# mbilos/stribor

Measured on AMD Instinct MI355X. Metric: log_prob samples/sec, D=64 8-layer affine-coupling, higher is better.
Workload: dtype f32

## Files before the change

stribor_amd/csrc/sx_flow_kernel.h:

```cpp
#pragma once
#include "sx_common.h"
#include "sx_flow_types.h"
#include "sx_cubic_core.h"
#include "sx_pointwise_core.h"
#include <stdlib.h>
#include <type_traits>

#define SX_HALF_LOG_2PI 0.91893853320467274178f

#ifdef SX_F16X3
#define SX_PREC_NS sx_f16x3
#else
#define SX_PREC_NS sx_f32x
#endif
namespace SX_PREC_NS {

__host__ __device__ static inline int sx_kmap(int r, int h) { return (r & 3) + 8 * (r >> 2) + 4 * h; }

extern __shared__ __attribute__((aligned(16))) float smem[];

typedef __attribute__((address_space(3))) void lds_void;

template <int NS>
struct tile {
// ... 419 lines not shown
#define SX_PIN_ACC(a) asm volatile("" : "+v"(a))
template <int NS, bool PIN = true, class F>
__device__ __forceinline__ void gemm_tile_pf(const char *wb, afr &cur, int next_off, const btile<NS> &b, tile<NS> &acc, F &&f) {
    afr nxt = cur;
    if (next_off >= 0) nxt = afr_load(wb, next_off);
    __builtin_amdgcn_sched_barrier(0);
#pragma unroll
    for (int s = 0; s < 2; ++s) {
        const h8 ah = __builtin_bit_cast(h8, cur.q[2 * s]), al = __builtin_bit_cast(h8, cur.q[2 * s + 1]);
#pragma unroll
        for (int n = 0; n < NS; ++n) { acc.v[n] = __builtin_amdgcn_mfma_f32_32x32x16_f16(al, b.hi[n][s], acc.v[n], 0, 0, 0); if constexpr (PIN) SX_PIN_ACC(acc.v[n]); }
        f(8 * s + 0); f(8 * s + 1); f(8 * s + 2);
        __builtin_amdgcn_sched_barrier(0);
#pragma unroll
        for (int n = 0; n < NS; ++n) { acc.v[n] = __builtin_amdgcn_mfma_f32_32x32x16_f16(ah, b.lo[n][s], acc.v[n], 0, 0, 0); if constexpr (PIN) SX_PIN_ACC(acc.v[n]); }
        f(8 * s + 3); f(8 * s + 4); f(8 * s + 5);
        __builtin_amdgcn_sched_barrier(0);
#pragma unroll
        for (int n = 0; n < NS; ++n) { acc.v[n] = __builtin_amdgcn_mfma_f32_32x32x16_f16(ah, b.hi[n][s], acc.v[n], 0, 0, 0); if constexpr (PIN) SX_PIN_ACC(acc.v[n]); }
        f(8 * s + 6); f(8 * s + 7);
        __builtin_amdgcn_sched_barrier(0);
    }
    cur = nxt;
}
__device__ __forceinline__ float pinned(float v) { asm volatile("" : "+v"(v)); return v; }
template <int NS, bool TRACK>
__device__ __forceinline__ void split_pair(const tile<NS> &c, u32x4 (&hi)[NS][2], u32x4 (&lo)[NS][2], int p, float &mx) {
#pragma unroll
    for (int n = 0; n < NS; ++n) {
        const float v0 = c.v[n][2 * p], v1 = c.v[n][2 * p + 1];
        if constexpr (TRACK) mx = rng_max(mx, v0, v1);
        const uint32_t ph = pk_f16(v0, v1);
        hi[n][p >> 2][p & 3] = ph;
        lo[n][p >> 2][p & 3] = pk_residual(ph, v0, v1);
    }
}
template <int NS>
__device__ __forceinline__ btile<NS> btile_of(const u32x4 (&hi)[NS][2], const u32x4 (&lo)[NS][2]) {
    btile<NS> b;
#pragma unroll
    for (int n = 0; n < NS; ++n)
#pragma unroll
        for (int s = 0; s < 2; ++s) { b.hi[n][s] = __builtin_bit_cast(h8, hi[n][s]); b.lo[n][s] = __builtin_bit_cast(h8, lo[n][s]); }
    return b;
}
template <int NS, int TX, int HT, int C0, int CT, int T0, int TT, bool REV>
__device__ __forceinline__ void coupling_affine_pf(tile<NS> (&xs)[TX], const wptr w, const dstep &st, float (&ldj)[NS],
                                                   rng_t &rg) {
    static_assert(CT == 2 && HT <= 2, "coupling_affine_pf: two conditioner tiles, hidden <= 64");
    constexpr int a2 = HT * CT * 1024 + HT * 32;
    constexpr int b2 = a2 + 2 * TT * HT * 1024;
    constexpr int bias1 = HT * CT * 1024;
    constexpr int NH = HT * CT, NO = 2 * TT * HT;
    auto off_of = [](int q) { return q < NH ? q * 1024 : (q < NH + NO ? a2 + (((q - NH) % (2 * TT)) * HT + (q - NH) / (2 * TT)) * 1024 : -1); };
    auto none = [](int) {};
    afr cur = afr_load(w.wb, 0);
    float mx = 0.f;
    u32x4 shi[NS][2], slo[NS][2];
    btile<NS> bsrc0 = make_btile_mx<NS>(xs[C0], mx);
    tile<NS> hid[HT];
    int q = 0;
    {
        tile<NS> acc = load_cfrag<NS>(w.cb, bias1);
        gemm_tile_pf<NS>(w.wb, cur, off_of(q + 1), bsrc0, acc, [&](int i) { if (!(i & 1)) split_pair<NS, true>(xs[C0 + 1], shi, slo, i >> 1, mx); });
        ++q;
        const btile<NS> bsrc1 = btile_of<NS>(shi, slo);
        gemm_tile_pf<NS>(w.wb, cur, off_of(q + 1), bsrc1, acc, none);
        ++q;
        hid[0] = acc;
        if constexpr (HT == 2) {
            tile<NS> acc1 = load_cfrag<NS>(w.cb, bias1 + 32);
            gemm_tile_pf<NS>(w.wb, cur, off_of(q + 1), bsrc0, acc1, [&](int i) {
                if (i & 1) return;
#pragma unroll
                for (int n = 0; n < NS; ++n) { hid[0].v[n][i] = pinned(fast_sig2(hid[0].v[n][i])); hid[0].v[n][i + 1] = pinned(fast_sig2(hid[0].v[n][i + 1])); }
            });
            ++q;
            gemm_tile_pf<NS>(w.wb, cur, off_of(q + 1), bsrc1, acc1, [&](int i) { if (!(i & 1)) split_pair<NS, false>(hid[0], shi, slo, i >> 1, mx); });
            ++q;
            hid[1] = acc1;
        }
        rng_note(rg, mx);
    }
    btile<NS> bh[HT];
    if constexpr (HT == 1) {
#pragma unroll
        for (int n = 0; n < NS; ++n)
#pragma unroll
            for (int r = 0; r < 16; r += 2) fast_sig2_pair(hid[0].v[n], r);
        bh[0] = make_btile<NS>(hid[0]);
    } else {
        bh[0] = btile_of<NS>(shi, slo);
    }
    f32x2 s[NS];
#pragma unroll
    for (int n = 0; n < NS; ++n) s[n] = f32x2{0.f, 0.f};
    tile<NS> out[2 * TT];
#pragma unroll
    for (int r = 0; r < 2 * TT; ++r) out[r] = load_cfrag<NS>(w.cb, b2 + r * 32);
    auto exp_rider = [&](tile<NS> &ls, int i) {
        if (i & 1) return;
#pragma unroll
        for (int n = 0; n < NS; ++n) {
            const float l0 = ls.v[n][i], l1 = ls.v[n][i + 1];
            s[n].x = pinned(s[n].x + l0);
            s[n].y = pinned(s[n].y + l1);
            ls.v[n][i] = pinned(__builtin_amdgcn_exp2f(l0));
            ls.v[n][i + 1] = pinned(__builtin_amdgcn_exp2f(l1));
        }
    };
    auto affine_rider = [&](tile<NS> &x, const tile<NS> &e, const tile<NS> &sh, int i) {
        if (i & 1) return;
#pragma unroll
        for (int n = 0; n < NS; ++n) {
            const f32x2 xv = {x.v[n][i], x.v[n][i + 1]}, sv = {sh.v[n][i], sh.v[n][i + 1]}, ev = {e.v[n][i], e.v[n][i + 1]};
            const f32x2 yv = REV ? pk_mul(pk_sub(xv, sv), ev) : pk_add(pk_mul(xv, ev), sv);
            x.v[n][i] = pinned(yv.x);
            x.v[n][i + 1] = pinned(yv.y);
        }
    };
#pragma unroll
    for (int k = 0; k < HT; ++k) {
#pragma unroll
        for (int r = 0; r < 2 * TT; ++r) {
            const bool last_k = k == HT - 1;
            gemm_tile_pf<NS>(w.wb, cur, off_of(q + 1), bh[k], out[r], [&](int i) {
                if (HT == 2 && k == 0) {
                    if (r == 0) {
                        if (!(i & 1)) {
#pragma unroll
                            for (int n = 0; n < NS; ++n) {
                                hid[HT - 1].v[n][i] = pinned(fast_sig2(hid[HT - 1].v[n][i]));
                                hid[HT - 1].v[n][i + 1] = pinned(fast_sig2(hid[HT - 1].v[n][i + 1]));
                            }
                        }
                    } else if (r <= 2) {
                        if ((i & 3) == 0) split_pair<NS, false>(hid[HT - 1], shi, slo, 4 * (r - 1) + (i >> 2), mx);
                    }
                }
                if (last_k) {
                    if (r & 1) exp_rider(out[r - 1], i);
                    else if (r >= 2) affine_rider(xs[T0 + r / 2 - 1], out[r - 2], out[r - 1], i);
                }
            });
            ++q;
            if (HT == 2 && k == 0 && r == 2) bh[1] = btile_of<NS>(shi, slo);
        }
    }
#pragma unroll
    for (int i = 0; i < 16; i += 2) affine_rider(xs[T0 + TT - 1], out[2 * TT - 2], out[2 * TT - 1], i);
#pragma unroll
    for (int n = 0; n < NS; ++n) ldj[n] += st.ldj_scale * (s[n].x + s[n].y);
}
#endif
template <int NS, int TX, int HT, int T0, int TT, bool REV>
__device__ __forceinline__ void coupling_affine_deep(tile<NS> (&xs)[TX], const tile<NS> (&hsrc)[HT], const wptr w,
                                                     const dstep &st, float (&ldj)[NS], rng_t &rg) {
    tile<NS> hid[HT];
    hidden_layer<NS, HT, HT, 0, HT, false>(hsrc, hid, w, 0, st.act, rg);
    constexpr int a2 = HT * HT * 1024 + HT * 32;
    constexpr int b2 = a2 + 2 * TT * HT * 1024;
    btile<NS> bh[HT];
#pragma unroll
    for (int m = 0; m < HT; ++m) bh[m] = make_btile<NS>(hid[m], rg);
    __builtin_amdgcn_sched_barrier(0);
    float s[NS];
#pragma unroll
    for (int n = 0; n < NS; ++n) s[n] = 0.f;
    const float sgn = REV ? -1.44269504088896341f : 1.44269504088896341f;
#pragma unroll
    for (int t = 0; t < TT; ++t) {
        tile<NS> ls = load_cfrag<NS>(w.cb, b2 + (2 * t) * 32);
        tile<NS> sh = load_cfrag<NS>(w.cb, b2 + (2 * t + 1) * 32);
#pragma unroll
        for (int m = 0; m < HT; ++m) {
            gemm_tile<NS>(w.wb, a2 + ((2 * t) * HT + m) * 1024, bh[m], ls);
            gemm_tile<NS>(w.wb, a2 + ((2 * t + 1) * HT + m) * 1024, bh[m], sh);
        }
        tile<NS> &x = xs[T0 + t];
#pragma unroll
        for (int n = 0; n < NS; ++n)
#pragma unroll
            for (int r = 0; r < 16; ++r) {
                s[n] += ls.v[n][r];
                const float e = __builtin_amdgcn_exp2f(ls.v[n][r] * sgn);
                x.v[n][r] = REV ? (x.v[n][r] - sh.v[n][r]) * e : x.v[n][r] * e + sh.v[n][r];
            }
    }
#pragma unroll
    for (int n = 0; n < NS; ++n) ldj[n] += st.ldj_scale * s[n];
}

template <int NS, int TX, int HT, int C0, int CT, int T0, int TT, bool REV, int PN>
__device__ __forceinline__ void coupling_affine_chunk(tile<NS> (&xs)[TX], tile<NS> (&pacc)[PN], const wptr w, const dstep &st,
                                                      float (&ldj)[NS], rng_t &rg) {
    tile<NS> hid[HT];
    hidden_layer<NS, TX, HT, C0, CT, true>(xs, hid, w, 0, SX_ACT_TANH_FOLDED, rg);
#pragma unroll
    for (int n = 0; n < NS; ++n)
#pragma unroll
        for (int r = 0; r < 16; r += 2) fast_sig2_pair(hid[HT - 1].v[n], r);
    btile<NS> bh[HT];
#pragma unroll
    for (int m = 0; m < HT; ++m) bh[m] = make_btile<NS>(hid[m]);
    __builtin_amdgcn_sched_barrier(0);
    constexpr int a2 = HT * CT * 1024 + HT * 32;
    constexpr int b2 = a2 + 2 * TT * HT * 1024;
    const bool first = st.pad & 1, last = st.pad & 2;
#pragma unroll
    for (int t = 0; t < 2 * TT; ++t) {
        tile<NS> acc = load_cfrag<NS>(w.cb, b2 + t * 32);
        if (!first) {
#pragma unroll
            for (int n = 0; n < NS; ++n)
#pragma unroll
                for (int r = 0; r < 16; ++r) acc.v[n][r] += pacc[t].v[n][r];
        }
#pragma unroll
        for (int m = 0; m < HT; ++m) gemm_tile<NS>(w.wb, a2 + (t * HT + m) * 1024, bh[m], acc);
        pacc[t] = acc;
    }
    if (last) {
#pragma unroll
        for (int t = 0; t < TT; ++t) {
            tile<NS> &x = xs[T0 + t];
#pragma unroll
            for (int n = 0; n < NS; ++n) {
                float s = 0.f;
#pragma unroll
                for (int r = 0; r < 16; ++r) {
                    const float l = pacc[2 * t].v[n][r], sh = pacc[2 * t + 1].v[n][r];
                    s += l;
                    const float e = __builtin_amdgcn_exp2f(l);
                    x.v[n][r] = REV ? (x.v[n][r] - sh) * e : x.v[n][r] * e + sh;
                }
                ldj[n] += st.ldj_scale * s;
            }
        }
    }
}
template <int NS, int TX, int HT, int C0, int CT, int T0, int TT, int PN>
__device__ __forceinline__ void coupling_affine_chunk_dispatch(tile<NS> (&xs)[TX], tile<NS> (&pacc)[PN], const wptr w, const dstep &st,
                                                               float (&ldj)[NS], rng_t &rg) {
    if (st.reverse) coupling_affine_chunk<NS, TX, HT, C0, CT, T0, TT, true>(xs, pacc, w, st, ldj, rg);
    else coupling_affine_chunk<NS, TX, HT, C0, CT, T0, TT, false>(xs, pacc, w, st, ldj, rg);
}

template <int TX, int HT, int C0>
__device__ __forceinline__ void wide_hidden(tile<1> (&xs)[TX], btile<1> (&bhp)[HT], const wptr w, rng_t &rg) {
    tile<1> hid[HT];
#ifdef SX_F16X3
    constexpr int CT = TX / 2;
    float mx = 0.f;
    btile<1> bsrc[CT];
#pragma unroll
    for (int c = 0; c < CT; ++c) bsrc[c] = make_btile_mx<1>(xs[C0 + c], mx);
    __builtin_amdgcn_sched_barrier(0);
    afr cura = afr_load(w.wb, 0);
    constexpr int bias = HT * CT * 1024;
#pragma unroll
    for (int m = 0; m < HT; ++m) {
        tile<1> acc = load_cfrag<1>(w.cb, bias + m * 32);
#pragma unroll
        for (int c = 0; c < CT; ++c) {
            const int qn = m * CT + c + 1;
            const int next_off = qn < HT * CT ? qn * 1024 : -1;
            if (m > 0 && c == 0)
                gemm_tile_pf<1, false>(w.wb, cura, next_off, bsrc[c], acc, [&](int i) { fast_sig2_pair(hid[m > 0 ? m - 1 : 0].v[0], i); });
            else
                gemm_tile_pf<1, false>(w.wb, cura, next_off, bsrc[c], acc, [](int) {});
        }
        hid[m] = acc;
    }
    rng_note(rg, mx);
#else
    hidden_layer<1, TX, HT, C0, TX / 2, true>(xs, hid, w, 0, SX_ACT_TANH_FOLDED, rg);
#endif
#pragma unroll
    for (int r = 0; r < 16; r += 2) fast_sig2_pair(hid[HT - 1].v[0], r);
#pragma unroll
    for (int m = 0; m < HT; ++m) bhp[m] = make_btile<1>(hid[m]);
}
template <int TX, int HT>
__device__ __forceinline__ void wide_affine_tile(tile<1> (&xs)[TX], const btile<1> (&bhp)[HT], const wptr w, const dstep &st, float &ldj) {
    tile<1> ls = load_cfrag<1>(w.cb, 2 * HT * 1024), sh = load_cfrag<1>(w.cb, 2 * HT * 1024 + 32);
#ifdef SX_F16X3
    afr cura = afr_load(w.wb, 0);
#pragma unroll
    for (int m = 0; m < HT; ++m) {
        gemm_tile_pf<1, false>(w.wb, cura, (HT + m) * 1024, bhp[m], ls, [](int) {});
        gemm_tile_pf<1, false>(w.wb, cura, m + 1 < HT ? (m + 1) * 1024 : -1, bhp[m], sh, [](int) {});
    }
#else
#pragma unroll
    for (int m = 0; m < HT; ++m) {
        gemm_tile<1>(w.wb, m * 1024, bhp[m], ls);
        gemm_tile<1>(w.wb, (HT + m) * 1024, bhp[m], sh);
    }
#endif
    float s = 0.f;
#pragma unroll
    for (int r = 0; r < 16; ++r) {
        s += ls.v[0][r];
        ls.v[0][r] = __builtin_amdgcn_exp2f(ls.v[0][r]);
    }
    const bool rev = st.reverse != 0;
// ... 369 lines not shown
            have_pf = false;
        }
        if (!from_frag)
#pragma unroll
        for (int n = 0; n < NS; ++n) {
#pragma unroll
            for (int t = 0; t < TX; ++t) {
                if (t < x_tiles) {
                    if (prog.identity_cols) {
#pragma unroll
                        for (int q = 0; q < 4; ++q) {
                            const int c = 32 * t + 8 * q + 4 * h;
                            f32x4 v = {0.f, 0.f, 0.f, 0.f};
                            if (c + 3 < dim) {
                                if (bf16) {
                                    const u16x4 u = *reinterpret_cast<const u16x4 *>(
                                        reinterpret_cast<const uint16_t *>(k.x) + lrow[n] * dim + c);
                                    v = f32x4{bf16_to_f32(u.x), bf16_to_f32(u.y), bf16_to_f32(u.z), bf16_to_f32(u.w)};
                                } else {
                                    constexpr bool NT_X = MODE == 3 || MODE == 10 || MODE == 12 || MODE == 13 || MODE == 18 || MODE == 19;
                                    if constexpr (NT_X) v = __builtin_nontemporal_load(reinterpret_cast<const f32x4 *>(reinterpret_cast<const float *>(k.x) + lrow[n] * dim + c));
                                    else v = *reinterpret_cast<const f32x4 *>(reinterpret_cast<const float *>(k.x) + lrow[n] * dim + c);
                                }
                            }
                            xs[t].v[n][4 * q + 0] = v.x; xs[t].v[n][4 * q + 1] = v.y;
                            xs[t].v[n][4 * q + 2] = v.z; xs[t].v[n][4 * q + 3] = v.w;
                        }
                    } else {
                        int cidx[16];
#pragma unroll
                        for (int r = 0; r < 16; ++r) cidx[r] = k.in_col[32 * t + sx_kmap(r, h)];
                        const int64_t rb = lrow[n] * (prog.pad ? prog.pad : dim);
                        if (bf16) {
                            uint16_t u[16];
#pragma unroll
                            for (int r = 0; r < 16; ++r) u[r] = reinterpret_cast<const uint16_t *>(k.x)[rb + (cidx[r] >= 0 ? cidx[r] : 0)];
#pragma unroll
                            for (int r = 0; r < 16; ++r) xs[t].v[n][r] = cidx[r] >= 0 ? bf16_to_f32(u[r]) : 0.f;
                        } else {
                            float u[16];
#pragma unroll
                            for (int r = 0; r < 16; ++r) u[r] = reinterpret_cast<const float *>(k.x)[rb + (cidx[r] >= 0 ? cidx[r] : 0)];
#pragma unroll
                            for (int r = 0; r < 16; ++r) xs[t].v[n][r] = cidx[r] >= 0 ? u[r] : 0.f;
                        }
                    }
                } else if constexpr (MODE == 4 || MODE == 11) {
                    if constexpr (TX == 2 || TX == 4 || TX == 8) {
                        const float gg = k.row_t[lrow[n]];
#pragma unroll
                        for (int r = 0; r < 16; ++r) xs[t].v[n][r] = -gg * xs[t - TX / 2].v[n][r];
                    }
                } else {
#pragma unroll
                    for (int r = 0; r < 16; ++r) {
                        const int c = 32 * (t - x_tiles) + sx_kmap(r, h);
                        float v = (k.latent != nullptr && c < prog.latent_dim) ? k.latent[lrow[n] * prog.latent_dim + c] : 0.f;
                        if constexpr (MODE == 15) {
                            if (c == prog.latent_dim && k.row_t != nullptr) v = k.row_t[lrow[n]];
                            if (c == prog.latent_dim + 1 && k.side != nullptr) v = k.side[lrow[n]];
                        }
                        xs[t].v[n][r] = v;
                    }
                }
            }
        }

        uint32_t ticket = 0;
        if (dyn && threadIdx.x == 0) ticket = atomicAdd(k.work, 1u);
        float ldj[NS];
#pragma unroll
        for (int n = 0; n < NS; ++n) ldj[n] = 0.f;
        float ldj_c = 0.f;
        rng_t rg;
        rg.bad = 0ull;
        rg.thr = k.redo != nullptr ? SX_REDO_ABOVE : SX_F16_MAX;
        tile<NS> hid[MODE == 1 ? HT : 1];
        constexpr bool LIN = MODE == 2 || MODE == 7 || MODE == 8;
        tile<NS> hidp[(MODE == 9 || MODE == 14 || MODE == 16 || MODE == 17) ? HT : 1];
        [[maybe_unused]] tile<NS> pacc[(MODE == 20 && TX >= 2 && TX <= 4) ? TX : 1];
        [[maybe_unused]] btile<1> bhp[(MODE == 20 && TX == 8) ? HT : 1];
        constexpr bool SIDE_OUT = MODE == 18 || MODE == 19;
        constexpr bool CUB = MODE == 12 || MODE == 13 || MODE == 19;
        constexpr bool RQ = MODE == 3 || MODE == 10 || MODE == 18 || CUB;
        constexpr bool RQDEEP = MODE == 10 || MODE == 13;
        constexpr bool MIX = MODE == 14 || MODE == 16 || MODE == 17;
        constexpr bool MIXC = MODE == 16, MIXQ = MODE == 17;
        btile<1> rq_bh[(RQ || MIX) ? HT : 1];
        std::conditional_t<(CUB || MIXC), cubic_elems, rqs_elems> rq_e;
        [[maybe_unused]] std::conditional_t<(MODE == 14), cubic_elems, int> rq_ec;
        [[maybe_unused]] bool rq_lean = true;

        for (int s = 0; s < n_steps; ++s) {
            const bool free_run = MODE == 11 && resident && !dyn && iter > 0;
            if (!free_run) {
                if constexpr (MODE == 4 && TX == 8) {
                    if (s > 0 && stores_young && head_counted) asm volatile("s_waitcnt vmcnt(63)" ::: "memory");
                    else asm volatile("s_waitcnt vmcnt(0)" ::: "memory");
                } else {
                    asm volatile("s_waitcnt vmcnt(0)" ::: "memory");
                }
                if (dyn && s == 0 && threadIdx.x == 0) slot[iter & 1] = ticket;
                __syncthreads();
                if (dyn && s == 0) next_chunk = (int64_t)gridDim.x + __builtin_amdgcn_readfirstlane(slot[iter & 1]);
            }
            const bool has_next_chunk = next_chunk < n_chunks;
            const dstep st = st_next;
            int wb_off = cur * buf_floats * 4 + lane * 16, cb_off = cur * buf_floats * 4 + (lane >> 5) * 64;
            asm volatile("" : "+v"(wb_off), "+v"(cb_off));
            constexpr bool DMA_LATE = (MODE == 7 || MODE == 8) && WB == 8;
            [[maybe_unused]] const uint32_t dma_off_now = dma_off, dma_floats_now = (s + 1 < n_steps || has_next_chunk) ? dma_floats : 0u;
            if constexpr (!DMA_LATE)
                if ((s + 1 < n_steps || has_next_chunk) && dma_floats && !resident)
                    stage_blob<WB>(k.blobs + dma_off, (cur ^ 1) * buf_floats, dma_floats);
            if constexpr (MODE == 11) {
                if (resident && s == 0 && k.frag_in != nullptr && has_next_chunk) {
                    const int64_t ngrp = next_chunk * WB + wave;
                    if (ngrp < ((n_rows + 31) >> 5)) {
                        const int64_t ngrp_s = __builtin_amdgcn_readfirstlane((int)ngrp);
                        const auto rsrc = __builtin_amdgcn_make_buffer_rsrc(const_cast<float *>(k.frag_in + ngrp_s * (TX * 4 * 64 * 4)), 0, TX * 4 * 1024, 0x00020000);
                        char *ldst = reinterpret_cast<char *>(smem + pf_base + __builtin_amdgcn_readfirstlane(wave) * 4096);
#pragma unroll
                        for (int i = 0; i < TX * 4; ++i)
                            __builtin_amdgcn_raw_ptr_buffer_load_lds(rsrc, (lds_void *)(ldst + i * 1024), 16, lane * 16, i * 1024, 0, 0);
                        const int64_t nrow = ngrp * 32 + (lane & 31);
                        gg_next = k.row_t[nrow < n_rows ? nrow : n_rows - 1];
                        have_pf = true;
                    }
                } else if (resident && s == 0 && k.frag_in == nullptr && has_next_chunk && dim == 32 * (TX / 2)) {
                    const int64_t ngrp = next_chunk * WB + wave;
                    if (ngrp < ((n_rows + 31) >> 5)) {
                        const int64_t nrow = ngrp * 32 + (lane & 31), nr = nrow < n_rows ? nrow : n_rows - 1;
                        const int64_t ngrp_s = __builtin_amdgcn_readfirstlane((int)ngrp);
                        const auto rsrc = __builtin_amdgcn_make_buffer_rsrc(const_cast<float *>(reinterpret_cast<const float *>(k.x) + ngrp_s * 32 * dim), 0, 0x7fffffff, 0x00020000);
                        const int voff = ((int)(nr - ngrp_s * 32) * dim + 4 * (lane >> 5)) * 4;
                        char *ldst = reinterpret_cast<char *>(smem + pf_base + __builtin_amdgcn_readfirstlane(wave) * 4096);
#pragma unroll
                        for (int i = 0; i < (TX / 2) * 4; ++i)
                            __builtin_amdgcn_raw_ptr_buffer_load_lds(rsrc, (lds_void *)(ldst + i * 1024), 16, voff, ((i >> 2) * 32 + (i & 3) * 8) * 4, 0, 0);
                        gg_next = k.row_t[nr];
                        have_pf = true;
                    }
                }
            }
            const int nxt = (s + 1 < n_steps) ? s + 1 : 0, nxt2 = (nxt + 1 < n_steps) ? nxt + 1 : 0;
            st_next = load_step(prog, nxt);
            dma_off = prog.steps[nxt2].blob_off;
            dma_floats = prog.steps[nxt2].blob_floats;

            const wptr w = wptr{reinterpret_cast<const char *>(smem) + wb_off, reinterpret_cast<const char *>(smem) + cb_off};
            [[maybe_unused]] float st_cur_const = st.ldj_const;
            if constexpr (MODE == 5 || MODE == 6) {
                if constexpr (TX >= 2) {
                    if (st.c0 == 0) coupling_affine<NS, TX, HT, 0, TX / 2, TX / 2, TX / 2, true, MODE == 5>(xs, w, st, ldj, rg);
                    else coupling_affine<NS, TX, HT, TX / 2, TX / 2, 0, TX / 2, true, MODE == 5>(xs, w, st, ldj, rg);
                }
            } else if constexpr (MODE == 11) {
#ifdef SX_F16X3
                if constexpr (TX == 4 && NS == 1 && HT <= 2) {
                    const float gg = gg11;
                    const bool live = row[0] < n_rows;
                    if (st.c0 == 0) coupling_affine_bwd_acc<HT, 0, 1>(xs, w, gg, live, WA, sel, rg);
                    else coupling_affine_bwd_acc<HT, 1, 0>(xs, w, gg, live, WA, sel, rg);
                }
#endif
            } else if ((MODE == 7 || MODE == 8) && st.kind == SX_STEP_COUPLING_AFFINE) {
                if constexpr (TX >= 2 && (MODE == 7 || MODE == 8)) {
#ifdef SX_F16X3
                    if constexpr (TX == 4 && HT <= 2) {
                        if (st.c0 == 0) coupling_affine_pf<NS, TX, HT, 0, TX / 2, TX / 2, TX / 2, MODE == 7>(xs, w, st, ldj, rg);
                        else coupling_affine_pf<NS, TX, HT, TX / 2, TX / 2, 0, TX / 2, MODE == 7>(xs, w, st, ldj, rg);
                    } else
#endif
                    if (st.c0 == 0) coupling_affine<NS, TX, HT, 0, TX / 2, TX / 2, TX / 2, true, MODE == 7>(xs, w, st, ldj, rg);
                    else coupling_affine<NS, TX, HT, TX / 2, TX / 2, 0, TX / 2, true, MODE == 7>(xs, w, st, ldj, rg);
                }
            } else if constexpr (MODE == 15) {
                if (st.kind == SX_STEP_COUPLING_TIME) {
                    float tv[NS];
#pragma unroll
                    for (int n = 0; n < NS; ++n) tv[n] = ((st.mask >> 8) & 1u) ? k.side[lrow[n]] : k.row_t[lrow[n]];
                    if (st.tt == TX) coupling_time_dispatch<NS, TX, HT, TX>(xs, w, st, ldj, rg, tv);
                    else if constexpr (TX >= 2) {
                        if (st.tt == TX / 2) coupling_time_dispatch<NS, TX, HT, TX / 2>(xs, w, st, ldj, rg, tv);
                        else if constexpr (TX >= 4) { if (st.tt == TX / 4) coupling_time_dispatch<NS, TX, HT, TX / 4>(xs, w, st, ldj, rg, tv); }
                    }
                }
            } else if constexpr (MODE == 4 && TX == 8) {
                if constexpr (NS == 1) {
                    float *srow = row[0] < n_rows ? k.side + ((int64_t)st.tt * ((n_rows + 31) >> 5) + (row[0] >> 5)) * (k.side_width * 32) + (row[0] & 31) : nullptr;
                    auto swap_tiles = [&](int a, int b) {
#pragma unroll
                        for (int r = 0; r < 16; ++r) { const float t_ = xs[a].v[0][r]; xs[a].v[0][r] = xs[b].v[0][r]; xs[b].v[0][r] = t_; }
                    };
#pragma unroll
                    for (int t = 0; t < TX; ++t)
#pragma unroll
                        for (int r = 0; r < 16; ++r) asm volatile("" : "+v"(xs[t].v[0][r]));
                    dstep stb;
                    wptr wb_ = w;
                    float *srow_b = nullptr;
                    auto second_half = [&]() {
                        cur ^= 1;
                        ++s;
                        if (stores_young) asm volatile("s_waitcnt vmcnt(63)" ::: "memory");
                        else asm volatile("s_waitcnt vmcnt(0)" ::: "memory");
                        asm volatile("s_waitcnt lgkmcnt(0)" ::: "memory");
                        __builtin_amdgcn_s_barrier();
                        stb = st_next;
                        if ((s + 1 < n_steps || has_next_chunk) && dma_floats) stage_blob<WB>(k.blobs + dma_off, (cur ^ 1) * buf_floats, dma_floats);
                        const int nb = (s + 1 < n_steps) ? s + 1 : 0, nb2 = (nb + 1 < n_steps) ? nb + 1 : 0;
                        st_next = load_step(prog, nb);
                        dma_off = prog.steps[nb2].blob_off;
                        dma_floats = prog.steps[nb2].blob_floats;
                        wb_ = make_wptr(cur * buf_floats, lane);
                        srow_b = row[0] < n_rows ? k.side + ((int64_t)stb.tt * ((n_rows + 31) >> 5) + (row[0] >> 5)) * (k.side_width * 32) + (row[0] & 31) : nullptr;
                    };
                    if (st.kind == SX_STEP_COUPLING_AFFINE_BWD_A) {
                        const float gg = gg_chunk;
                        const bool high = st.c0 != 0;
                        if (high) { swap_tiles(0, 2); swap_tiles(1, 3); swap_tiles(4, 6); swap_tiles(5, 7); }
                        tile<1> keep[HT + 4];
                        coupling_affine_bwd_a<4, HT, 0, 2, 2, 2>(xs, w, gg, srow, lane, rg, keep);
                        second_half();
                        coupling_affine_bwd_b<4, HT, 0, 2, 2, 2>(xs, wb_, srow_b, lane, rg, keep);
                        if (high) { swap_tiles(0, 2); swap_tiles(1, 3); swap_tiles(4, 6); swap_tiles(5, 7); }
                        head_counted = HT >= 2;
                    } else if (st.kind == SX_STEP_LINEAR_BWD) {
                        linear_bwd_half<4, 0>(xs, w, srow, 32 * st.t0, st.reverse != 0, lane, rg);
                        second_half();
                        linear_bwd_half<4, 4>(xs, wb_, srow_b, 32 * stb.t0, stb.reverse != 0, lane, rg);
                        head_counted = true;
                    }
                }
            } else
            switch (st.kind) {
                case SX_STEP_COUPLING_AFFINE:
                    if constexpr (RQ || MODE == 7 || MODE == 8 || TX == 8) break;
                    if constexpr (TX >= 2) {
                        if (st.ct == TX / 2 && st.c0 == 0 && st.t0 == TX / 2) {
                            coupling_affine_dispatch<NS, TX, HT, 0, TX / 2, TX / 2, TX / 2>(xs, w, st, ldj, rg);
                            break;
                        }
                        if (st.ct == TX / 2 && st.c0 == TX / 2 && st.t0 == 0) {
                            coupling_affine_dispatch<NS, TX, HT, TX / 2, TX / 2, 0, TX / 2>(xs, w, st, ldj, rg);
                            break;
                        }
                    }
                    coupling_affine_dispatch<NS, TX, HT, 0, TX, 0, TX>(xs, w, st, ldj, rg);
                    break;
                case SX_STEP_AFFINE_CONST:
                    if constexpr (MODE != 7 && MODE != 8) affine_const<NS, TX>(xs, w, st, x_tiles, ldj);
                    break;
                case SX_STEP_MLP_HIDDEN:
                    if constexpr (MODE == 1) hidden_layer<NS, TX, HT, 0, TX, false>(xs, hid, w, 0, st.act, rg);
                    break;
                case SX_STEP_MLP_INPUT:
                    if constexpr (MODE == 1 && TX <= HT) {
#pragma unroll
                        for (int m = 0; m < HT; ++m) {
                            if (m < TX) hid[m] = xs[m];
                            else {
#pragma unroll
                                for (int n = 0; n < NS; ++n)
#pragma unroll
                                    for (int r = 0; r < 16; ++r) hid[m].v[n][r] = 0.f;
                            }
                        }
                    }
                    break;
                case SX_STEP_CPL_HIDDEN:
                    if constexpr (MIX && NS == 1) {
                        if constexpr (TX >= 2) {
                            if (st.ct == TX / 2 && st.c0 == 0) hidden_layer<1, TX, HT, 0, TX / 2, false>(xs, hidp, w, 0, st.act, rg);
                            else if (st.ct == TX / 2) hidden_layer<1, TX, HT, TX / 2, TX / 2, false>(xs, hidp, w, 0, st.act, rg);
                            else hidden_layer<1, TX, HT, 0, TX, false>(xs, hidp, w, 0, st.act, rg);
                        } else {
                            hidden_layer<1, TX, HT, 0, TX, false>(xs, hidp, w, 0, st.act, rg);
                        }
#pragma unroll
                        for (int m = 0; m < HT; ++m) rq_bh[m] = make_btile<1>(hidp[m], rg);
                        break;
                    }
                    if constexpr (RQDEEP && NS == 1) {
                        tile<1> hd[HT];
                        if constexpr (TX >= 2) {
                            if (st.ct == TX / 2 && st.c0 == 0) hidden_layer<1, TX, HT, 0, TX / 2, false>(xs, hd, w, 0, st.act, rg);
                            else if (st.ct == TX / 2) hidden_layer<1, TX, HT, TX / 2, TX / 2, false>(xs, hd, w, 0, st.act, rg);
                            else hidden_layer<1, TX, HT, 0, TX, false>(xs, hd, w, 0, st.act, rg);
                        } else {
                            hidden_layer<1, TX, HT, 0, TX, false>(xs, hd, w, 0, st.act, rg);
                        }
#pragma unroll
                        for (int m = 0; m < HT; ++m) rq_bh[m] = make_btile<1>(hd[m], rg);
                    }
                    if constexpr (MODE == 9) {
                        if constexpr (TX >= 2) {
                            if (st.ct == TX / 2 && st.c0 == 0) { hidden_layer<NS, TX, HT, 0, TX / 2, false>(xs, hidp, w, 0, st.act, rg); break; }
                            if (st.ct == TX / 2 && st.c0 == TX / 2) { hidden_layer<NS, TX, HT, TX / 2, TX / 2, false>(xs, hidp, w, 0, st.act, rg); break; }
                        }
                        hidden_layer<NS, TX, HT, 0, TX, false>(xs, hidp, w, 0, st.act, rg);
                    }
                    break;
                case SX_STEP_CPL_HIDDEN2:
                    if constexpr (MIX && NS == 1) {
                        tile<1> nh[HT];
// ... 542 lines not shown
```

Baseline: 3.216 billion.

## Add hand-scheduled affine coupling path interleaving MFMA with split-f16 conversion work

Adds a specialised affine-coupling routine for TX==2, HT==2 under the f16x3 precision path. It interleaves the three-pass split-f16 MFMAs with the conversion of inputs into hi/lo halves, the activation math, weight fragment loads and the exp/affine epilogue, separated by scheduling barriers. The goal is to hide the VALU and LDS latency behind matrix instructions instead of running the phases back to back. The cost is a large amount of fragile hand-scheduled code, and it only takes effect when SX_F16X3 is defined and the tile shape matches.

```diff
diff --git a/stribor_amd/csrc/sx_flow_kernel.h b/stribor_amd/csrc/sx_flow_kernel.h
--- a/stribor_amd/csrc/sx_flow_kernel.h
+++ b/stribor_amd/csrc/sx_flow_kernel.h
@@ -595,6 +595,170 @@
 #pragma unroll
     for (int n = 0; n < NS; ++n) ldj[n] += st.ldj_scale * (s[n].x + s[n].y);
 }
+struct ks_frag { h8 ah, al; };
+__device__ __forceinline__ ks_frag ks_load(const char *wb, int a_off, int s) {
+    const u32x4 ahu = *reinterpret_cast<const u32x4 *>(wb + (a_off + (2 * s) * 256) * 4);
+    const u32x4 alu = *reinterpret_cast<const u32x4 *>(wb + (a_off + (2 * s + 1) * 256) * 4);
+    return ks_frag{__builtin_bit_cast(h8, ahu), __builtin_bit_cast(h8, alu)};
+}
+__device__ __forceinline__ uint32_t pinned_u(uint32_t v) { asm volatile("" : "+v"(v)); return v; }
+template <int LO, int HI, class F>
+__device__ __forceinline__ void ks_ops(F &&f) {
+#pragma unroll
+    for (int j = LO; j < HI; ++j) f(j);
+}
+template <int NS, class R1, class R2, class R3>
+__device__ __forceinline__ void ks_group(tile<NS> &acc, const ks_frag &a, const u32x4 (&hi)[NS][2], const u32x4 (&lo)[NS][2], int s,
+                                         R1 &&r1, R2 &&r2, R3 &&r3) {
+#pragma unroll
+    for (int n = 0; n < NS; ++n) { acc.v[n] = __builtin_amdgcn_mfma_f32_32x32x16_f16(a.al, __builtin_bit_cast(h8, hi[n][s]), acc.v[n], 0, 0, 0); SX_PIN_ACC(acc.v[n]); }
+    __builtin_amdgcn_sched_barrier(0);
+    r1();
+    __builtin_amdgcn_sched_barrier(0);
+#pragma unroll
+    for (int n = 0; n < NS; ++n) { acc.v[n] = __builtin_amdgcn_mfma_f32_32x32x16_f16(a.ah, __builtin_bit_cast(h8, lo[n][s]), acc.v[n], 0, 0, 0); SX_PIN_ACC(acc.v[n]); }
+    __builtin_amdgcn_sched_barrier(0);
+    r2();
+    __builtin_amdgcn_sched_barrier(0);
+#pragma unroll
+    for (int n = 0; n < NS; ++n) { acc.v[n] = __builtin_amdgcn_mfma_f32_32x32x16_f16(a.ah, __builtin_bit_cast(h8, hi[n][s]), acc.v[n], 0, 0, 0); SX_PIN_ACC(acc.v[n]); }
+    __builtin_amdgcn_sched_barrier(0);
+    r3();
+    __builtin_amdgcn_sched_barrier(0);
+}
+template <int NS, int C0, int T0, bool REV>
+__device__ __forceinline__ void coupling_affine_ks(tile<NS> (&xs)[2], const wptr w, const dstep &st, float (&ldj)[NS], rng_t &rg) {
+    constexpr int bias1 = 2 * 1024;
+    constexpr int a2 = bias1 + 2 * 32;
+    constexpr int b2 = a2 + 4 * 1024;
+    static_assert(NS == 1, "coupling_affine_ks: one sample tile per wave");
+    const tile<NS> &src = xs[C0];
+    tile<NS> &x = xs[T0];
+    float mx;
+    float t0[NS][4], t1[NS][4];
+    u32x4 xhi[NS][2], xlo[NS][2], phi[NS][2], plo[NS][2];
+    f32x2 sum[NS];
+#pragma unroll
+    for (int n = 0; n < NS; ++n) sum[n] = f32x2{0.f, 0.f};
+    auto aside = [] { asm volatile("s_nop 5"); };
+    auto x_op = [&](int j) {
+        const int q = 4 * (j / 20), k = j % 20;
+        const int p = q + (k < 8 ? k / 2 : (k < 16 ? (k - 8) / 2 : k - 16));
+#pragma unroll
+        for (int n = 0; n < NS; ++n) {
+            const float v0 = src.v[n][2 * p], v1 = src.v[n][2 * p + 1];
+            const uint32_t ph = xhi[n][p >> 2][p & 3];
+            if (k < 8 && !(k & 1)) {
+                if (j == 0) asm("v_max3_f32 %0, 0, |%1|, |%2|" : "=v"(mx) : "v"(v0), "v"(v1));
+                else mx = rng_max(mx, v0, v1);
+                mx = pinned(mx);
+            } else if (k < 8) xhi[n][p >> 2][p & 3] = pinned_u(pk_f16(v0, v1));
+            else if (k < 16 && !(k & 1)) { asm("v_fma_mix_f32 %0, %1, -1.0, %2 op_sel_hi:[1,0,0]" : "=v"(t0[n][p & 3]) : "v"(ph), "v"(v0)); t0[n][p & 3] = pinned(t0[n][p & 3]); }
+            else if (k < 16) { asm("v_fma_mix_f32 %0, %1, -1.0, %2 op_sel:[1,0,0] op_sel_hi:[1,0,0]" : "=v"(t1[n][p & 3]) : "v"(ph), "v"(v1)); t1[n][p & 3] = pinned(t1[n][p & 3]); }
+            else xlo[n][p >> 2][p & 3] = pinned_u(pk_f16(t0[n][p & 3], t1[n][p & 3]));
+        }
+    };
+    auto s_op = [&](float (&h)[NS][16], int j) {
+        const int k = j % 12, r = 4 * (j / 12) + (k & 3);
+#pragma unroll
+        for (int n = 0; n < NS; ++n) {
+            const float v = h[n][r];
+            h[n][r] = pinned(k < 4 ? __builtin_amdgcn_exp2f(v) : (k < 8 ? v + 1.0f : __builtin_amdgcn_rcpf(v)));
+        }
+    };
+    auto p_op = [&](const float (&h)[NS][16], int j) {
+        const int q = 4 * (j / 16), k = j % 16;
+        const int p = q + (k < 4 ? k : (k < 12 ? (k - 4) / 2 : k - 12));
+#pragma unroll
+        for (int n = 0; n < NS; ++n) {
+            const float v0 = h[n][2 * p], v1 = h[n][2 * p + 1];
+            const uint32_t ph = phi[n][p >> 2][p & 3];
+            if (k < 4) phi[n][p >> 2][p & 3] = pinned_u(pk_f16(v0, v1));
+            else if (k < 12 && !(k & 1)) { asm("v_fma_mix_f32 %0, %1, -1.0, %2 op_sel_hi:[1,0,0]" : "=v"(t0[n][p & 3]) : "v"(ph), "v"(v0)); t0[n][p & 3] = pinned(t0[n][p & 3]); }
+            else if (k < 12) { asm("v_fma_mix_f32 %0, %1, -1.0, %2 op_sel:[1,0,0] op_sel_hi:[1,0,0]" : "=v"(t1[n][p & 3]) : "v"(ph), "v"(v1)); t1[n][p & 3] = pinned(t1[n][p & 3]); }
+            else plo[n][p >> 2][p & 3] = pinned_u(pk_f16(t0[n][p & 3], t1[n][p & 3]));
+        }
+    };
+    tile<NS> ls, sh;
+    auto e_op = [&](int j) {
+        const int p = j / 4, k = j % 4;
+#pragma unroll
+        for (int n = 0; n < NS; ++n) {
+            if (k == 0) sum[n].x = pinned(sum[n].x + ls.v[n][2 * p]);
+            else if (k == 1) sum[n].y = pinned(sum[n].y + ls.v[n][2 * p + 1]);
+            else ls.v[n][2 * p + k - 2] = pinned(__builtin_amdgcn_exp2f(ls.v[n][2 * p + k - 2]));
+        }
+    };
+    auto f_op = [&](int p) {
+#pragma unroll
+        for (int n = 0; n < NS; ++n) {
+            const f32x2 xv = {x.v[n][2 * p], x.v[n][2 * p + 1]}, sv = {sh.v[n][2 * p], sh.v[n][2 * p + 1]};
+            const f32x2 ev = {ls.v[n][2 * p], ls.v[n][2 * p + 1]};
+            const f32x2 yv = REV ? pk_mul(pk_sub(xv, sv), ev) : pk_add(pk_mul(xv, ev), sv);
+            x.v[n][2 * p] = yv.x;
+            x.v[n][2 * p + 1] = yv.y;
+        }
+    };
+    tile<NS> c0, c1;
+    float h0[NS][16], h1[NS][16];
+    ks_frag f, g;
+    ks_ops<0, 5>(x_op);
+    __builtin_amdgcn_sched_barrier(0);
+    c0 = load_cfrag<NS>(w.cb, bias1);
+    f = ks_load(w.wb, 0, 0);
+    __builtin_amdgcn_sched_barrier(0);
+    ks_ops<5, 20>(x_op);
+    __builtin_amdgcn_sched_barrier(0);
+    ks_group<NS>(c0, f, xhi, xlo, 0, [&] { ks_ops<20, 24>(x_op); }, [&] { ks_ops<24, 28>(x_op); },
+                 [&] { c1 = load_cfrag<NS>(w.cb, bias1 + 32); g = ks_load(w.wb, 1024, 0); ks_ops<28, 31>(x_op); });
+    ks_group<NS>(c1, g, xhi, xlo, 0, [&] { ks_ops<31, 34>(x_op); }, [&] { ks_ops<34, 37>(x_op); },
+                 [&] { f = ks_load(w.wb, 0, 1); ks_ops<37, 40>(x_op); rng_note(rg, mx); });
+    ks_group<NS>(c0, f, xhi, xlo, 1, aside, aside, [&] { aside(); g = ks_load(w.wb, 1024, 1); });
+#pragma unroll
+    for (int n = 0; n < NS; ++n)
+#pragma unroll
+        for (int r = 0; r < 16; ++r) h0[n][r] = c0.v[n][r];
+    ks_group<NS>(c1, g, xhi, xlo, 1, [&] { ks_ops<0, 3>([&](int j) { s_op(h0, j); }); }, [&] { ks_ops<3, 8>([&](int j) { s_op(h0, j); }); },
+                 [&] { f = ks_load(w.wb, a2, 0); ks_ops<8, 11>([&](int j) { s_op(h0, j); }); });
+#pragma unroll
+    for (int n = 0; n < NS; ++n)
+#pragma unroll
+        for (int r = 0; r < 16; ++r) h1[n][r] = c1.v[n][r];
+    ks_ops<11, 24>([&](int j) { s_op(h0, j); });
+    ks_ops<0, 8>([&](int j) { p_op(h0, j); });
+    __builtin_amdgcn_sched_barrier(0);
+    ls = load_cfrag<NS>(w.cb, b2);
+    __builtin_amdgcn_sched_barrier(0);
+    ks_ops<8, 16>([&](int j) { p_op(h0, j); });
+    __builtin_amdgcn_sched_barrier(0);
+    ks_group<NS>(ls, f, phi, plo, 0, [&] { ks_ops<24, 27>([&](int j) { s_op(h0, j); }); }, [&] { ks_ops<27, 32>([&](int j) { s_op(h0, j); }); },
+                 [&] { sh = load_cfrag<NS>(w.cb, b2 + 32); g = ks_load(w.wb, a2 + 2 * 1024, 0); ks_ops<32, 35>([&](int j) { s_op(h0, j); }); });
+    ks_group<NS>(sh, g, phi, plo, 0, [&] { ks_ops<35, 38>([&](int j) { s_op(h0, j); }); }, [&] { ks_ops<38, 42>([&](int j) { s_op(h0, j); }); },
+                 [&] { f = ks_load(w.wb, a2, 1); ks_ops<42, 46>([&](int j) { s_op(h0, j); }); });
+    ks_ops<46, 48>([&](int j) { s_op(h0, j); });
+    ks_ops<16, 32>([&](int j) { p_op(h0, j); });
+    __builtin_amdgcn_sched_barrier(0);
+    ks_group<NS>(ls, f, phi, plo, 1, [&] { ks_ops<0, 3>([&](int j) { s_op(h1, j); }); }, [&] { ks_ops<3, 8>([&](int j) { s_op(h1, j); }); },
+                 [&] { g = ks_load(w.wb, a2 + 2 * 1024, 1); ks_ops<8, 11>([&](int j) { s_op(h1, j); }); });
+    ks_group<NS>(sh, g, phi, plo, 1, [&] { ks_ops<11, 14>([&](int j) { s_op(h1, j); }); }, [&] { ks_ops<14, 18>([&](int j) { s_op(h1, j); }); },
+                 [&] { f = ks_load(w.wb, a2 + 1024, 0); ks_ops<18, 22>([&](int j) { s_op(h1, j); }); });
+    ks_ops<22, 24>([&](int j) { s_op(h1, j); });
+    ks_ops<0, 16>([&](int j) { p_op(h1, j); });
+    __builtin_amdgcn_sched_barrier(0);
+    ks_group<NS>(ls, f, phi, plo, 0, [&] { ks_ops<24, 27>([&](int j) { s_op(h1, j); }); }, [&] { ks_ops<27, 32>([&](int j) { s_op(h1, j); }); },
+                 [&] { g = ks_load(w.wb, a2 + 3 * 1024, 0); ks_ops<32, 35>([&](int j) { s_op(h1, j); }); });
+    ks_group<NS>(sh, g, phi, plo, 0, [&] { ks_ops<35, 38>([&](int j) { s_op(h1, j); }); }, [&] { ks_ops<38, 42>([&](int j) { s_op(h1, j); }); },
+                 [&] { f = ks_load(w.wb, a2 + 1024, 1); ks_ops<42, 46>([&](int j) { s_op(h1, j); }); });
+    ks_ops<46, 48>([&](int j) { s_op(h1, j); });
+    ks_ops<16, 32>([&](int j) { p_op(h1, j); });
+    __builtin_amdgcn_sched_barrier(0);
+    ks_group<NS>(ls, f, phi, plo, 1, aside, aside, [&] { aside(); g = ks_load(w.wb, a2 + 3 * 1024, 1); });
+    ks_group<NS>(sh, g, phi, plo, 1, [&] { ks_ops<0, 4>(e_op); }, [&] { ks_ops<4, 8>(e_op); }, [&] { ks_ops<8, 12>(e_op); });
+    ks_ops<12, 32>(e_op);
+    ks_ops<0, 8>(f_op);
+#pragma unroll
+    for (int n = 0; n < NS; ++n) ldj[n] += st.ldj_scale * (sum[n].x + sum[n].y);
+}
 #endif
 template <int NS, int TX, int HT, int T0, int TT, bool REV>
 __device__ __forceinline__ void coupling_affine_deep(tile<NS> (&xs)[TX], const tile<NS> (&hsrc)[HT], const wptr w,
@@ -1270,6 +1434,12 @@
             [[maybe_unused]] float st_cur_const = st.ldj_const;
             if constexpr (MODE == 5 || MODE == 6) {
                 if constexpr (TX >= 2) {
+#ifdef SX_F16X3
+                    if constexpr (TX == 2 && HT == 2) {
+                        if (st.c0 == 0) coupling_affine_ks<NS, 0, 1, MODE == 5>(xs, w, st, ldj, rg);
+                        else coupling_affine_ks<NS, 1, 0, MODE == 5>(xs, w, st, ldj, rg);
+                    } else
+#endif
                     if (st.c0 == 0) coupling_affine<NS, TX, HT, 0, TX / 2, TX / 2, TX / 2, true, MODE == 5>(xs, w, st, ldj, rg);
                     else coupling_affine<NS, TX, HT, TX / 2, TX / 2, 0, TX / 2, true, MODE == 5>(xs, w, st, ldj, rg);
                 }
```

After: 3.264 billion, median of 6. 1.5% higher.
